# NVlabs/DREAM

Measured on AMD Instinct MI355X. Metric: frames/s DREAM-vgg-q 400x400 b=128 inference, higher is better.
Workload: dtype f32

## Files before the change

dream_amd/csrc/conv_wino4.hip:

```cpp
#include <type_traits>
#include <stdlib.h>
#include <dream_cdna4.h>
#include "common.h"
#include "pack_device.h"
#include "../../include/dream_hip.h"

#ifndef DREAM_W4_DIAG
#define DREAM_W4_DIAG 0
#endif
#ifndef DREAM_W4_STORE
#define DREAM_W4_STORE buffer_store_f32
#endif
#ifndef DREAM_W4_MIDBARRIER
#define DREAM_W4_MIDBARRIER 0
#endif
#ifndef DREAM_W4_STAGGER_N
#define DREAM_W4_STAGGER_N 0
#define DREAM_W4_STAGGER_PCT 0
#endif
#ifndef DREAM_W4_WAUX
#define DREAM_W4_WAUX 0
#endif
#ifndef DREAM_W4_XAUX
#define DREAM_W4_XAUX 0
#endif
#ifndef DREAM_W4_STAG_LX
#define DREAM_W4_STAG_LX 0
#endif
#ifndef DREAM_W4_RUNNING_WOFF
#define DREAM_W4_RUNNING_WOFF 1
#endif
#ifndef DREAM_W4_SETPRIO
#define DREAM_W4_SETPRIO 0
#endif

namespace {

struct Wino4Params {
    const float *x;
    const float *u;
    const float *scale;
    const float *shift;
    const float *residual;
    float *y;
    float *y_full;
    int B, H, W, Cin, Cout, CoutPad;
    int TY, TX;
    int ntiles;
    int nblk, blk_per_xcd;
    unsigned long long magic_tpi, magic_tx;
    int flags;
    int out_scale, out_oy, out_ox;
    int in_scale, in_oy, in_ox;
    int stagger_n, stagger_unit;
    int ymap;
};

constexpr int W4T = 16;
constexpr int W4P = 36;
#ifndef DREAM_W4_RING
#define DREAM_W4_RING 8
#endif
#ifndef DREAM_W4_NARROW_RING
#define DREAM_W4_NARROW_RING 18
#endif
#ifndef DREAM_W4_PAT_RING
#define DREAM_W4_PAT_RING 10
#endif
#ifndef DREAM_W4_PAT_S1OFF
#define DREAM_W4_PAT_S1OFF 8
#endif


template <bool NARROW>
struct W4Cfg {
    static constexpr int NW = NARROW ? 4 : 8;
    static constexpr int K = NARROW ? 8 : 16;
    static constexpr int Q = K / 4;
    static constexpr int KS = K / 4;
    static constexpr int PAD = 16 * NW;
    static constexpr int VPS = NARROW ? W4T * K : W4T * K + 16;
    static constexpr int VB = W4P * VPS;
    static constexpr int SROW = NARROW ? 14 : 25;
    static constexpr int QS = NARROW ? 7 : 6;
    static constexpr int SB = W4T * 6 * SROW * 4;
    static constexpr int RING = NARROW ? DREAM_W4_NARROW_RING : DREAM_W4_RING;
    static constexpr int AHEAD = RING - 2;
    static_assert(72 % RING == 0, "the weight ring must divide two chunks' positions");
    static constexpr bool PAIRS = NARROW && DREAM_W4_NARROW_PAIRS;
    static_assert(!PAIRS || RING % 2 == 0, "a ring of whole pairs");
    using vec = std::conditional_t<NARROW, f32x2, f32x4>;
};
template <bool NARROW>
DREAM_DEVICE int v4_slot(int q, int t) { return NARROW ? q ^ ((t >> 3) & 1) : q ^ ((t >> 2) & 2); }

DREAM_DEVICE f32x4 fma4(float c, f32x4 a, f32x4 b) {
    f32x4 r;
#pragma unroll
    for (int k = 0; k < 4; ++k) r[k] = __builtin_fmaf(c, a[k], b[k]);
    return r;
}

DREAM_DEVICE f32x4 sub4(f32x4 y, f32x4 x) { return pk_sub4(y, x); }
DREAM_DEVICE f32x4 bt_row(int j, const f32x4 *d) {
    switch (j) {
        case 0: return fma4(-2.0f, d[2], fma4(1.5f, sub4(d[3], d[1]), d[0] + d[4]));
        case 1: return fma4(2.5f, d[3], fma4(0.5f, d[2], sub4(d[4], d[1])));
        case 2: return fma4(0.5f, d[3], fma4(-2.5f, d[2], d[4] + d[1]));
        case 3: return fma4(2.0f, sub4(d[3], d[1]), sub4(d[4], d[2]));
        case 4: return fma4(-0.5f, sub4(d[3], d[1]), sub4(d[4], d[2]));
        default: return fma4(-2.0f, d[3], fma4(1.5f, sub4(d[4], d[2]), d[1] + d[5]));
    }
}

DREAM_DEVICE constexpr bool pat4_row_active(int pat, int i) { return pat == 0 || (((pat - 1) >> 1) == 0 ? i <= 4 : i >= 1); }
DREAM_DEVICE constexpr bool pat4_col_active(int pat, int j) { return pat == 0 || (((pat - 1) & 1) == 0 ? j <= 4 : j >= 1); }
DREAM_DEVICE constexpr bool pat4_active(int pat, int pp) { return pat4_row_active(pat, pp / 6) && pat4_col_active(pat, pp % 6); }
DREAM_DEVICE constexpr int pat4_count(int pat) { return pat == 0 ? 36 : 25; }
struct Pat4Table { int pos[36]; };
constexpr Pat4Table pat4_table(int pat) {
    Pat4Table t = {};
    int n = 0;
    for (int pp = 0; pp < 36; ++pp)
        if (pat4_active(pat, pp)) t.pos[n++] = pp;
    return t;
}
template <int PAT>
struct Pat4 { static constexpr Pat4Table table = pat4_table(PAT); };
#define pat4_pos(PAT, k) (Pat4<PAT>::table.pos[k])

template <int MODE, bool NARROW, int PAT = 0>
__global__ void __launch_bounds__(64 * W4Cfg<NARROW>::NW, 2) conv_wino4_kernel(const Wino4Params p) {
    using C = W4Cfg<NARROW>;
    using vec = typename C::vec;
    constexpr int W4K = C::K, W4NW = C::NW, V4PS = C::VPS, V4B = C::VB, S4ROW = C::SROW;
    constexpr int NPOS = pat4_count(PAT);
    constexpr int W4_RING = PAT ? DREAM_W4_PAT_RING : C::RING, W4_AHEAD = W4_RING - 2;
    static_assert((2 * NPOS) % W4_RING == 0, "the weight ring must divide two chunks' positions");
    DREAM_DYNAMIC_LDS(float, sV);
    const int tid = threadIdx.x;
    const int lane = tid & 63;
    const int wave = wave_index();
    const int item_id = wave * 48 + (lane < 48 ? lane : lane - 16);

    const int xcd = (int)(blockIdx.x & 7), J = (int)(gridDim.x >> 3);
    const int part = p.ymap ? xcd / p.ymap : xcd;
    const int blk_hi = (part + 1) * p.blk_per_xcd;
    const int blk_end = blk_hi < p.nblk ? blk_hi : p.nblk;
    int tb = part * p.blk_per_xcd + (int)(blockIdx.x >> 3);
    if (tb >= blk_end) return;
    const int n0 = (p.ymap ? xcd % p.ymap : (int)blockIdx.y) * (16 * W4NW);
    if (p.stagger_n > 1) {
        const unsigned w = blockIdx.x + blockIdx.y * gridDim.x;
        const int naps = (int)((w * 2654435761u >> 16) % (unsigned)p.stagger_n) * p.stagger_unit;
        for (int i = 0; i < naps; ++i) __builtin_amdgcn_s_sleep(127);
    }
    const int tiles_per_img = p.TY * p.TX;
    const int Si = PAT ? p.in_scale : 1;
    const size_t img_floats = (size_t)(Si * p.H) * (Si * p.W) * p.Cin;

    const int q1 = item_id % C::Q, r1 = (item_id / C::Q) % 6, t1 = (item_id / C::Q) / 6;
    const int s1_off = ((t1 * 6 + r1) * S4ROW + C::QS * q1) * 4;
    const int q2 = item_id % C::Q;
    const int j2 = NARROW ? (item_id >> 3) % 6 : (item_id >> 2) % 6;
    const int t2 = NARROW ? 4 * (item_id / 48) + ((item_id >> 1) & 3) : (item_id >> 2) / 6;
    const int s2_off = ((t2 * 6) * S4ROW + C::QS * q2 + j2) * 4;
    const int v2_off = j2 * V4PS + t2 * W4K + 4 * v4_slot<NARROW>(q2, t2);

    unsigned goff0;
    int item1 = t1 | (r1 << 8) | (q1 << 16);
    auto plan_item = [&](int tile0, int b0) {
        asm volatile("" : "+v"(item1));
        const int t = item1 & 255, r = (item1 >> 8) & 255, q = (item1 >> 16) & 255;
        const int tau = tile0 + t;
        const bool tv = tau < p.ntiles;
        const int b = div_magic40(tau, p.magic_tpi), rem = tau - b * tiles_per_img;
        const int ty = div_magic40(rem, p.magic_tx), tx = rem - ty * p.TX;
        const int gy = 4 * ty - 1 + r, x0 = 4 * tx - 1;
        const bool rok = tv & ((unsigned)gy < (unsigned)p.H);
        goff0 = PAT ? (unsigned)(((((b - b0) * Si * p.H + Si * gy + p.in_oy) * (Si * p.W) + Si * x0 + p.in_ox) * p.Cin + 4 * q) * 4)
                    : (unsigned)(((((b - b0) * p.H + gy) * p.W + x0) * p.Cin + 4 * q) * 4);
        item1 &= 0xffffff;
#pragma unroll
        for (int c = 0; c < 6; ++c) item1 |= (rok & ((unsigned)(x0 + c) < (unsigned)p.W)) ? (1 << (24 + c)) : 0;
    };
    const unsigned px_in = (unsigned)(Si * p.Cin * 4);
    auto item_offset = [&](int c) {
        if (DREAM_W4_DIAG & 16) {
            unsigned o = BUFFER_OOB;
            asm volatile("" : "+v"(o));
            return o;
        }
        return (item1 >> (24 + c)) & 1 ? goff0 + (unsigned)c * px_in : BUFFER_OOB;
    };
    auto block_tile0 = [&](int blk) { return blk < blk_end ? blk * W4T : p.ntiles; };
    auto block_xbuf = [&](int b0) {
        return make_buffer(p.x + (size_t)b0 * img_floats, ((size_t)(p.B - b0) * img_floats) * sizeof(float));
    };

    const int lt = lane & 15, lg = lane >> 4;
    const int a_off = NARROW ? lt * W4K + 4 * v4_slot<NARROW>(lg >> 1, lt) + 2 * (lg & 1) : lt * W4K + 4 * v4_slot<NARROW>(lg, lt);
    const unsigned b_lane = C::PAIRS ? (unsigned)(((wave * 16 + lt) * 16 + 4 * lg) * 4) : (unsigned)(((wave * 16 + lt) * W4K + C::KS * lg) * 4);
    const unsigned u_pos_stride = (unsigned)(p.CoutPad * W4K * 4);
    const BufferRsrc ubuf = make_buffer(p.u + (size_t)n0 * W4K, ((size_t)((p.Cin / W4K) * W4P + C::AHEAD) * p.CoutPad - (size_t)n0) * W4K * sizeof(float));

    f32x4 acc[W4P];
    const int nchunks = p.Cin / W4K;
    if (DREAM_W4_SETPRIO && wave >= W4NW / 2) __builtin_amdgcn_s_setprio(1);

    constexpr int BSTEP = C::PAIRS ? 2 : 1;
    std::conditional_t<C::PAIRS, f32x4, vec> bq[W4_RING / BSTEP];
    auto load_u = [&](unsigned soff) {
        if constexpr (C::PAIRS) return buffer_load_x4(ubuf, b_lane, soff);
        else if constexpr (NARROW) return buffer_load_x2(ubuf, b_lane, soff);
        else return buffer_load_x4_aux<DREAM_W4_WAUX>(ubuf, b_lane, soff);
    };
#pragma unroll
    for (int k = 0; k < W4_AHEAD; k += BSTEP) bq[k / BSTEP] = load_u((unsigned)pat4_pos(PAT, k) * u_pos_stride);
    unsigned woff = (unsigned)W4_AHEAD * u_pos_stride;
    DREAM_OPAQUE_SGPR(woff);

    f32x4 *const sV4 = (f32x4 *)sV;
    vec *const sVa = (vec *)sV;
    int vrd[2], vwr[2], s1p = (2 * V4B + s1_off) / 4, s2p = (2 * V4B + s2_off) / 4;
#pragma unroll
    for (int h = 0; h < 2; ++h) {
        vrd[h] = (h * V4B + a_off) / C::KS;
        vwr[h] = (h * V4B + v2_off) / 4;
        asm volatile("" : "+v"(vrd[h]), "+v"(vwr[h]));
    }
    asm volatile("" : "+v"(s1p), "+v"(s2p));
    f32x4 d[6];
    auto pass1_piece = [&](int j) { sV4[s1p + j] = bt_row(j, d); };
    auto pass2_read = [&](int r) { d[r] = sV4[s2p + r * S4ROW]; };
    auto pass2_piece = [&](int i, int h) { if (pat4_row_active(PAT, i)) sV4[vwr[h] + i * (6 * V4PS / 4)] = bt_row(i, d); };

    vec a[2][2];
    auto read_a = [&](int set, int k, int h) {
        const int p0 = pat4_pos(PAT, k), p1 = pat4_pos(PAT, k + 1 < NPOS ? k + 1 : k);
        if constexpr (NARROW) {
            a[set][0] = lds_read_unmerged(sVa + vrd[h] + p0 * V4PS / C::KS);
            a[set][1] = lds_read_unmerged(sVa + vrd[h] + p1 * V4PS / C::KS);
        } else {
            a[set][0] = sVa[vrd[h] + p0 * V4PS / C::KS];
            if (k + 1 < NPOS) a[set][1] = sVa[vrd[h] + p1 * V4PS / C::KS];
        }
    };

    int tile0 = block_tile0(tb);
    int b0 = div_magic40(tile0, p.magic_tpi);
    BufferRsrc xbuf = block_xbuf(b0);
    plan_item(tile0, b0);
#pragma unroll
    for (int c = 0; c < 6; ++c) d[c] = buffer_load_x4(xbuf, item_offset(c), 0u);
#pragma unroll
    for (int j = 0; j < 6; ++j) pass1_piece(j);
    __syncthreads();
#pragma unroll
    for (int r = 0; r < 6; ++r) pass2_read(r);
#pragma unroll
    for (int i = 0; i < 6; ++i) pass2_piece(i, 0);
    __syncthreads();

    auto chunk = [&](auto ph_tag, auto stag_tag, bool last, int c, int tile0n, int b0n) __attribute__((always_inline)) {
        constexpr int PH = decltype(ph_tag)::value;
        constexpr int STAG = decltype(stag_tag)::value;
#ifndef DREAM_W4_S1
#define DREAM_W4_S1 10
#define DREAM_W4_S2 13
#define DREAM_W4_LX 3
#endif
        constexpr int NSLOT = (NPOS + 1) / 2;
        constexpr int S1 = PAT ? NSLOT - DREAM_W4_PAT_S1OFF : DREAM_W4_S1, S2 = PAT ? S1 + 3 : DREAM_W4_S2;
        constexpr int LX = PAT ? 1 : DREAM_W4_LX;
        constexpr int LX0 = STAG ? DREAM_W4_STAG_LX : 0;
        static_assert(LX0 + LX <= S1, "the patch loads must be issued before pass 1");
        const unsigned coff = last ? 0u : (unsigned)((c + 1) * W4K * 4);
        const int cnext = last ? 0 : (c + 1) * W4P;
        if (PH == 1 && last) xbuf = block_xbuf(b0n);
        read_a(0, 0, PH);
        __builtin_amdgcn_sched_barrier(0);
#pragma unroll
        for (int s = 0; s < NSLOT; ++s) {
            const int k0 = 2 * s;
            const bool two = k0 + 1 < NPOS;
            const int pp = pat4_pos(PAT, k0), pp1 = pat4_pos(PAT, two ? k0 + 1 : k0);
            auto load_b = [&](int half) {
                if ((DREAM_W4_DIAG & 2) || (half && !two)) return;
                if (C::PAIRS && half) return;
                const int kn = k0 + half + W4_AHEAD;
                if constexpr (PAT == 0 && DREAM_W4_RUNNING_WOFF && !(DREAM_W4_DIAG & 32)) {
                    if (kn == NPOS && last) woff = 0u;
                    bq[(PH * NPOS + kn) % W4_RING / BSTEP] = load_u(woff);
                    woff += BSTEP * u_pos_stride;
                    DREAM_OPAQUE_SGPR(woff);
                } else {
                    const int spos = kn >= NPOS ? cnext + pat4_pos(PAT, kn - NPOS) : c * W4P + pat4_pos(PAT, kn);
                    bq[(PH * NPOS + kn) % W4_RING / BSTEP] = load_u((DREAM_W4_DIAG & 32) ? 0u : (unsigned)spos * u_pos_stride);
                }
            };
            auto load_x = [&](int col) { if (!(DREAM_W4_DIAG & 1)) d[col] = buffer_load_x4_aux<DREAM_W4_XAUX>(xbuf, item_offset(col), (DREAM_W4_DIAG & 64) ? 0u : coff); };
            auto pair = [&](int r) {
                const int i0 = (PH * NPOS + k0) % W4_RING, i1 = (PH * NPOS + k0 + 1) % W4_RING;
                if constexpr (C::PAIRS) {
                    acc[pp] = mfma_f32_16x16x4(a[s & 1][0][r], bq[i0 / 2][r], acc[pp]);
                    acc[pp1] = mfma_f32_16x16x4(a[s & 1][1][r], bq[i0 / 2][2 + r], acc[pp1]);
                } else {
                    acc[pp] = mfma_f32_16x16x4(a[s & 1][0][r], bq[i0][r], acc[pp]);
                    if (two) acc[pp1] = mfma_f32_16x16x4(a[s & 1][1][r], bq[i1][r], acc[pp1]);
                }
                __builtin_amdgcn_sched_barrier(0);
            };
            auto after = [&](int k) {
                if (k == 0) {
                    load_b(0);
                    if (s + 1 < NSLOT) read_a((s + 1) & 1, k0 + 2, PH);
                    if (PH == 1 && s == 0 && last) plan_item(tile0n, b0n);
                    if (s >= LX0 && s < LX0 + LX) { for (int c2 = 0; c2 < 3 / LX; ++c2) load_x((6 / LX) * (s - LX0) + c2); }
                    if (!(DREAM_W4_DIAG & 8) && s >= S1 && s < S1 + 3) pass1_piece(2 * (s - S1));
                    if (!(DREAM_W4_DIAG & 8) && s == S2) { pass2_read(0); pass2_read(1); }
                    if (!(DREAM_W4_DIAG & 8) && s > S2 && s <= S2 + 3) pass2_piece(2 * (s - S2 - 1), 1 - PH);
                } else if (k == 1) {
                    load_b(1);
                    if (s >= LX0 && s < LX0 + LX) { for (int c2 = 3 / LX; c2 < 6 / LX; ++c2) load_x((6 / LX) * (s - LX0) + c2); }
                    if (!(DREAM_W4_DIAG & 8) && s == S2) { pass2_read(2); pass2_read(3); }
                } else if (k == 2) {
                    if (!(DREAM_W4_DIAG & 8) && s >= S1 && s < S1 + 3) pass1_piece(2 * (s - S1) + 1);
                    if (!(DREAM_W4_DIAG & 8) && s == S2) { pass2_read(4); pass2_read(5); }
                    if (!(DREAM_W4_DIAG & 8) && s > S2 && s <= S2 + 3) pass2_piece(2 * (s - S2 - 1) + 1, 1 - PH);
                }
            };
            if constexpr (NARROW) {
                pair(0);
                after(0);
                after(1);
                pair(1);
                after(2);
            } else {
                pair(0);
                after(0);
                pair(1);
                after(1);
                pair(2);
                after(2);
                pair(3);
            }
            if (s == S1 + 2 && !(DREAM_W4_DIAG & 4)) {
                if (DREAM_W4_MIDBARRIER) __syncthreads();
                __builtin_amdgcn_sched_barrier(0);
            }
        }
        if (!(DREAM_W4_DIAG & 4)) __syncthreads();
    };
    const std::integral_constant<int, 0> ph0{};
    const std::integral_constant<int, 1> ph1{};

    constexpr bool pool = MODE == 1 || MODE == 4, both = MODE == 4, has_res = MODE == 2 || MODE == 3, mask = MODE == 3;
    auto epilogue = [&](auto site_tag, int tile0e, int b0e) {
        if (DREAM_W4_DIAG & 128) {
#pragma unroll
            for (int pp = 0; pp < W4P; ++pp)
                if (pat4_active(PAT, pp)) asm volatile("" :: "v"(acc[pp]));
            return;
        }
        const auto &e = *DREAM_KERNARG_SITE(p, decltype(site_tag)::value);
        const bool relu = (e.flags & DREAM_CONV_RELU) != 0;
        const bool late = MODE == 2 && (e.flags & DREAM_CONV_RES_AFTER_RELU) != 0;
        const int Ho = pool ? e.H / 2 : e.H, Wo = pool ? e.W / 2 : e.W, So = e.out_scale;
        const size_t out_img = (size_t)(So * Ho) * (So * Wo) * e.Cout;
        const unsigned px_b = (unsigned)(So * e.Cout * 4), row_b = (unsigned)(So * So * Wo * e.Cout * 4);
        const int ln = lane_id();
        const int lt = ln & 15, lg = ln >> 4;
        const int col = n0 + wave * 16 + lt;
        const bool cok = col < e.Cout;
        const float sc = (e.scale != nullptr && cok) ? e.scale[col] : 1.0f;
        const float sh = (e.shift != nullptr && cok) ? e.shift[col] : 0.0f;
        const BufferRsrc ybuf = make_buffer(e.y + (size_t)b0e * out_img, (DREAM_W4_DIAG & 256) ? 0 : (size_t)(e.B - b0e) * out_img * sizeof(float));
        const BufferRsrc rbuf = make_buffer(has_res ? e.residual + (size_t)b0e * out_img : e.y,
                                            has_res ? (size_t)(e.B - b0e) * out_img * sizeof(float) : 0);
        const size_t full_img = (size_t)e.H * e.W * e.Cout;
        const unsigned fpx_b = (unsigned)(e.Cout * 4), frow_b = (unsigned)(e.W * e.Cout * 4);
        const BufferRsrc fbuf = make_buffer(both ? e.y_full + (size_t)b0e * full_img : e.y, both ? (size_t)(e.B - b0e) * full_img * sizeof(float) : 0);
        const int tau0 = tile0e + lg * 4;
        int b = div_magic40(tau0, p.magic_tpi);
        const int rem = tau0 - b * tiles_per_img;
        int ty = div_magic40(rem, p.magic_tx), tx = rem - ty * p.TX;
        constexpr int NS = pool ? 2 : 4;
        unsigned basef[2][2];
        int limf[2][2];
        unsigned base4[2][2];
        int lim4[2][2];
        constexpr int FULL = pool ? 0x33 : 0xff;
#pragma unroll
        for (int rp = 0; rp < 2; ++rp)
#pragma unroll
            for (int h = 0; h < 2; ++h) {
                const bool tok = cok & ((tau0 + 2 * rp + h) < p.ntiles);
                const int oy = NS * ty, ox = NS * tx;
                base4[rp][h] = (unsigned)(((((b - b0e) * So * Ho + So * oy + e.out_oy) * (So * Wo) + So * ox + e.out_ox) * e.Cout + col) * 4);
                int m = 0;
#pragma unroll
                for (int i = 0; i < NS; ++i) m |= ((oy + i) < Ho ? 1 << i : 0) | ((ox + i) < Wo ? 16 << i : 0);
                lim4[rp][h] = tok ? m : 0;
                if (both) {
                    basef[rp][h] = (unsigned)(((((b - b0e) * e.H + 4 * ty) * e.W + 4 * tx) * e.Cout + col) * 4);
                    int mf = 0;
#pragma unroll
                    for (int i = 0; i < 4; ++i) mf |= ((4 * ty + i) < e.H ? 1 << i : 0) | ((4 * tx + i) < e.W ? 16 << i : 0);
                    limf[rp][h] = tok ? mf : 0;
                }
                const bool wrap_x = (tx + 1 == p.TX);
                const bool wrap_y = wrap_x & (ty + 1 == p.TY);
                tx = wrap_x ? 0 : tx + 1;
                ty = wrap_y ? 0 : (wrap_x ? ty + 1 : ty);
                b += wrap_y ? 1 : 0;
            }
        auto out_off4 = [&](int rp, int h, int i, int jj) {
            const bool inb = ((lim4[rp][h] >> i) & (lim4[rp][h] >> (4 + jj)) & 1) != 0;
            return inb ? base4[rp][h] + (unsigned)i * row_b + (unsigned)jj * px_b : BUFFER_OOB;
        };
        bool interior4[2];
#pragma unroll
        for (int rp = 0; rp < 2; ++rp) interior4[rp] = wave_all((lim4[rp][0] == FULL) & (lim4[rp][1] == FULL));
        auto load_col0 = [&](int rp, float (&r)[2][4]) {
            if (interior4[rp]) {
#pragma unroll
                for (int h = 0; h < 2; ++h)
#pragma unroll
                    for (int i = 0; i < 4; ++i) r[h][i] = buffer_load_f32(rbuf, base4[rp][h], (unsigned)i * row_b);
            } else {
#pragma unroll
                for (int h = 0; h < 2; ++h)
#pragma unroll
                    for (int i = 0; i < 4; ++i) r[h][i] = buffer_load_f32(rbuf, out_off4(rp, h, i, 0), 0u);
            }
        };
        float r0[2][4], r0n[2][4];
        if (has_res) load_col0(0, r0);
#pragma unroll
        for (int rp = 0; rp < 2; ++rp) {
            const unsigned (&base)[2] = base4[rp];
            auto out_off = [&](int h, int i, int jj) { return out_off4(rp, h, i, jj); };
            const bool all_interior = interior4[rp];
            auto fm = [](float c, f32x2 x, f32x2 y) { return __builtin_elementwise_fma(f32x2{c, c}, x, y); };
            f32x2 sA[6][4];
#pragma unroll
            for (int i = 0; i < 6; ++i) {
                f32x2 m[6];
#pragma unroll
                for (int j = 0; j < 6; ++j)
                    m[j] = pat4_active(PAT, 6 * i + j) ? f32x2{acc[6 * i + j][2 * rp], acc[6 * i + j][2 * rp + 1]} : f32x2{0.0f, 0.0f};
                const f32x2 t1 = pk_sub2(m[1], m[2]), t2 = m[1] + m[2];
                sA[i][0] = (m[0] + t2) + (m[3] + m[4]);
                sA[i][1] = fm(-2.0f, m[4], fm(0.5f, m[3], t1));
                sA[i][2] = fm(4.0f, m[4], fm(0.25f, m[3], t2));
                sA[i][3] = fm(-8.0f, m[4], fm(0.125f, m[3], t1)) + m[5];
            }
            auto finish = [&](float v, float rv) {
                if (has_res) v = mask ? (rv > 0.0f ? v : 0.0f) : (late ? v : v + rv);
                const float vr = fmaxf(v, 0.0f);
                v = relu ? vr : v;
                return (MODE == 2 && late) ? v + rv : v;
            };
            auto columns = [&](auto interior_tag, auto &rcur) {
                constexpr bool interior = decltype(interior_tag)::value;
                auto voff = [&](int h, int i, int j2) { return interior ? base[h] : out_off(h, i, j2); };
                auto soff = [&](int i, int j2) { return interior ? (unsigned)i * row_b + (unsigned)j2 * px_b : 0u; };
                float keep[2][2];
#pragma unroll
                for (int jj = 0; jj < 4; ++jj) {
                    float rnext[2][4];
                    if (has_res && jj == 3 && rp == 0) load_col0(1, r0n);
                    if (has_res && jj + 1 < 4) {
#pragma unroll
                        for (int h = 0; h < 2; ++h)
#pragma unroll
                            for (int i = 0; i < 4; ++i) rnext[h][i] = buffer_load_f32(rbuf, voff(h, i, jj + 1), soff(i, jj + 1));
                    }
                    const f32x2 t1 = pk_sub2(sA[1][jj], sA[2][jj]), t2 = sA[1][jj] + sA[2][jj];
                    f32x2 o4[4];
                    o4[0] = (sA[0][jj] + t2) + (sA[3][jj] + sA[4][jj]);
                    o4[1] = fm(-2.0f, sA[4][jj], fm(0.5f, sA[3][jj], t1));
                    o4[2] = fm(4.0f, sA[4][jj], fm(0.25f, sA[3][jj], t2));
                    o4[3] = fm(-8.0f, sA[4][jj], fm(0.125f, sA[3][jj], t1)) + sA[5][jj];
#pragma unroll
                    for (int i = 0; i < 4; ++i) o4[i] = o4[i] * f32x2{sc, sc} + f32x2{sh, sh};
#pragma unroll
                    for (int h = 0; h < 2; ++h) {
                        if (pool) {
                            float v[4];
#pragma unroll
                            for (int i = 0; i < 4; ++i) v[i] = finish(o4[i][h], 0.0f);
                            if (both) {
#pragma unroll
                                for (int i = 0; i < 4; ++i) {
                                    const bool inb = ((limf[rp][h] >> i) & (limf[rp][h] >> (4 + jj)) & 1) != 0;
                                    DREAM_W4_STORE(fbuf, v[i], inb ? basef[rp][h] + (unsigned)i * frow_b + (unsigned)jj * fpx_b : BUFFER_OOB, 0u);
                                }
                            }
                            if ((jj & 1) == 0) {
                                keep[h][0] = fmaxf(v[0], v[1]);
                                keep[h][1] = fmaxf(v[2], v[3]);
                            } else {
                                DREAM_W4_STORE(ybuf, fmaxf(keep[h][0], fmaxf(v[0], v[1])), voff(h, 0, jj >> 1), soff(0, jj >> 1));
                                DREAM_W4_STORE(ybuf, fmaxf(keep[h][1], fmaxf(v[2], v[3])), voff(h, 1, jj >> 1), soff(1, jj >> 1));
                            }
                        } else {
#pragma unroll
                            for (int i = 0; i < 4; ++i)
                                DREAM_W4_STORE(ybuf, finish(o4[i][h], has_res ? rcur[h][i] : 0.0f), voff(h, i, jj), soff(i, jj));
                        }
                    }
                    if (has_res && jj + 1 < 4) {
#pragma unroll
                        for (int h = 0; h < 2; ++h)
#pragma unroll
                            for (int i = 0; i < 4; ++i) rcur[h][i] = rnext[h][i];
                    }
                }
            };
            if (all_interior) columns(std::true_type{}, r0);
            else columns(std::false_type{}, r0);
            if (has_res && rp == 0) {
#pragma unroll
                for (int h = 0; h < 2; ++h)
#pragma unroll
                    for (int i = 0; i < 4; ++i) r0[h][i] = r0n[h][i];
            }
        }
    };

    auto run_blocks = [&](auto stag_tag) __attribute__((always_inline)) {
        while (true) {
            const int tile0n = block_tile0(tb + J);
            const int b0n = div_magic40(tile0n, p.magic_tpi);
            const f32x4 zero = {0.0f, 0.0f, 0.0f, 0.0f};
#pragma unroll
            for (int pp = 0; pp < W4P; ++pp)
                if (pat4_active(PAT, pp)) acc[pp] = zero;
            for (int c = 0; c < nchunks; c += 2) {
                chunk(ph0, stag_tag, false, c, tile0n, b0n);
                chunk(ph1, stag_tag, c + 2 == nchunks, c + 1, tile0n, b0n);
            }
            epilogue(stag_tag, tile0, b0);
            tb += J;
            if (tb >= blk_end) break;
            tile0 = tile0n;
            b0 = b0n;
        }
    };
    if constexpr (!NARROW && PAT == 0 && DREAM_W4_STAG_LX > 0) {
        if (wave >= W4NW / 2) run_blocks(std::integral_constant<int, 1>{});
        else run_blocks(std::integral_constant<int, 0>{});
    } else {
        run_blocks(std::integral_constant<int, 0>{});
    }
}

static_assert(W4Cfg<false>::K == 16 && W4Cfg<false>::PAD == 128 && W4Cfg<true>::K == 8 && W4Cfg<true>::PAD == 64 && W4P == 36,
              "pack_device.h assumes 16-channel chunks padded to 128 rows / 8-channel chunks padded to 64 rows, 36 positions");
__global__ void __launch_bounds__(256) wino4_pack_kernel(const float *w, float *u, int Cout, int Cin, int mode) {
    dream_pack::winograd4(w, u, Cout, Cin, mode, (int)blockIdx.x, (int)gridDim.x);
}

int g_max_workgroups4 = 0;
int g_stagger_n4 = -1, g_stagger_pct4 = 0;
int g_ymap4 = -1;

bool narrow_rows(int rows) { return rows <= W4Cfg<true>::PAD; }
struct PackShape { int k, rows_pad, ahead; };
PackShape pack_shape(int rows) {
    if (narrow_rows(rows)) return {W4Cfg<true>::K, W4Cfg<true>::PAD, W4Cfg<true>::AHEAD};
    return {W4Cfg<false>::K, (rows + W4Cfg<false>::PAD - 1) / W4Cfg<false>::PAD * W4Cfg<false>::PAD, W4Cfg<false>::AHEAD};
}

template <int MODE, bool NARROW, int PAT = 0>
int launch_wino4(const Wino4Params &p, void *stream) {
    using C = W4Cfg<NARROW>;
    void (*kernel)(const Wino4Params) = conv_wino4_kernel<MODE, NARROW, PAT>;
    const size_t lds = ((size_t)2 * C::VB + C::SB) * sizeof(float);
    if (dream_allow_full_lds((const void *)kernel)) return 2;
    const int ny = (p.Cout + 16 * C::NW - 1) / (16 * C::NW);
    const int resident = g_max_workgroups4 > 0 ? g_max_workgroups4 : (NARROW ? 512 : 256);
    Wino4Params q = p;
    dim3 grid;
    if (g_ymap4 && !NARROW && (ny == 2 || ny == 4) && resident >= 64 && p.nblk >= resident) {
        q.ymap = ny;
        q.blk_per_xcd = (p.nblk + 8 / ny - 1) / (8 / ny);
        grid = dim3((unsigned)(resident / 8 * 8), 1u);
    } else {
        int gx = resident / ny / 8 * 8;
        if (gx < 8) gx = 8;
        if (gx > (p.nblk + 7) / 8 * 8) gx = (p.nblk + 7) / 8 * 8;
        grid = dim3((unsigned)gx, (unsigned)ny);
    }
    hipLaunchKernelGGL(kernel, grid, dim3(64 * C::NW), lds, (hipStream_t)stream, q);
    DREAM_LAUNCH_OK();
    return 0;
}

template <bool NARROW>
int launch_wino4_mode(const Wino4Params &p, int mode, void *stream) {
    switch (mode) {
        case 0: return launch_wino4<0, NARROW>(p, stream);
        case 1: return launch_wino4<1, NARROW>(p, stream);
        case 2: return launch_wino4<2, NARROW>(p, stream);
        case 4: return launch_wino4<4, NARROW>(p, stream);
        default: return launch_wino4<3, NARROW>(p, stream);
    }
}

}

extern "C" size_t dream_conv3x3_winograd4_weight_floats(int rows, int cols) {
    const PackShape ps = pack_shape(rows);
    return ((size_t)(cols / ps.k) * W4P + ps.ahead) * ps.rows_pad * ps.k;
}

extern "C" int dream_conv3x3_winograd4_set_channel_block_pinning(int on) {
    DREAM_REQUIRE(on >= -1 && on <= 1, "winograd F(4x4): pinning %d", on);
    g_ymap4 = on;
    return 0;
}

extern "C" int dream_conv3x3_winograd4_set_stagger(int phases, int percent) {
    DREAM_REQUIRE(phases <= 1024 && percent >= 0 && percent <= 400, "winograd F(4x4): stagger %d phases over %d %%", phases, percent);
    g_stagger_n4 = phases < 0 ? -1 : (phases > 1 ? phases : 0);
    g_stagger_pct4 = percent;
    return 0;
}

extern "C" int dream_conv3x3_winograd4_set_max_workgroups(int n) {
    DREAM_REQUIRE(n >= 0, "winograd F(4x4): max workgroups %d", n);
    g_max_workgroups4 = n;
    return 0;
}

extern "C" int dream_pack_conv3x3_winograd4_weight(const float *w_oihw, float *u, int Cout, int Cin, int mode, void *stream) {
    DREAM_REQUIRE(w_oihw && u && Cout > 0 && Cin > 0 && (mode == 0 || mode == 1), "winograd F(4x4) pack: bad arguments");
    const int rows = mode == 0 ? Cout : Cin, cols = mode == 0 ? Cin : Cout;
    const PackShape ps = pack_shape(rows);
    DREAM_REQUIRE(cols % (2 * ps.k) == 0, "winograd F(4x4) pack: %d input channels, must be a multiple of %d", cols, 2 * ps.k);
    const size_t total = (size_t)(cols / ps.k) * ps.rows_pad * ps.k;
    size_t grid = (total + 255) / 256;
    if (grid > 4096) grid = 4096;
    hipLaunchKernelGGL(wino4_pack_kernel, dim3((unsigned)grid), dim3(256), 0, (hipStream_t)stream, w_oihw, u, Cout, Cin, mode);
    DREAM_LAUNCH_OK();
    if (dream_zero_words(u + (size_t)(cols / ps.k) * W4P * ps.rows_pad * ps.k, (size_t)ps.ahead * ps.rows_pad * ps.k * sizeof(float), (hipStream_t)stream))
        return 2;
    return 0;
}

namespace {

int wino4_setup(Wino4Params &p, const float *x, const float *u_packed, const float *scale, const float *shift, const float *residual,
                float *y, int B, int H, int W, int Cin, int Cout, int flags, int out_scale, int in_scale = 1) {
    DREAM_REQUIRE(x && u_packed && y, "winograd F(4x4) conv: null pointer");
    DREAM_REQUIRE(B > 0 && H > 0 && W > 0 && Cin > 0 && Cout > 0, "winograd F(4x4) conv: bad shape B=%d H=%d W=%d Cin=%d Cout=%d", B, H, W, Cin, Cout);
    const PackShape ps = pack_shape(Cout);
    DREAM_REQUIRE(Cin % (2 * ps.k) == 0, "winograd F(4x4) conv: Cin=%d must be a multiple of %d", Cin, 2 * ps.k);
    const size_t span_imgs = (size_t)W4T / ((size_t)((H + 3) / 4) * ((W + 3) / 4)) + 2;
    DREAM_REQUIRE(span_imgs * in_scale * in_scale * H * W * (size_t)Cin * sizeof(float) < ((size_t)1 << 31) &&
                  span_imgs * out_scale * out_scale * H * W * (size_t)Cout * sizeof(float) < ((size_t)1 << 31),
                  "winograd F(4x4) conv: image too large for 32-bit offsets");
    p.x = x; p.u = u_packed; p.scale = scale; p.shift = shift; p.residual = residual; p.y = y; p.y_full = nullptr;
    p.B = B; p.H = H; p.W = W; p.Cin = Cin; p.Cout = Cout;
    p.CoutPad = Cout <= ps.rows_pad ? ps.rows_pad : (Cout + ps.rows_pad - 1) / ps.rows_pad * ps.rows_pad;
    DREAM_REQUIRE(((size_t)(Cin / ps.k) * W4P + ps.ahead) * (size_t)p.CoutPad * ps.k * sizeof(float) < ((size_t)1 << 31), "winograd F(4x4) conv: weights too large");
    p.TY = (H + 3) / 4; p.TX = (W + 3) / 4;
    const long ntiles = (long)B * p.TY * p.TX;
    DREAM_REQUIRE(ntiles < ((long)1 << 24), "winograd F(4x4) conv: %ld tiles, the tile decomposition handles < 2^24", ntiles);
    p.ntiles = (int)ntiles;
    p.nblk = (p.ntiles + W4T - 1) / W4T;
    p.blk_per_xcd = (p.nblk + 7) / 8;
    p.magic_tpi = (((unsigned long long)1 << 40) + (unsigned long long)(p.TY * p.TX) - 1) / (unsigned long long)(p.TY * p.TX);
    p.magic_tx = (((unsigned long long)1 << 40) + (unsigned long long)p.TX - 1) / (unsigned long long)p.TX;
    p.flags = flags;
    p.out_scale = out_scale; p.out_oy = 0; p.out_ox = 0;
    p.in_scale = in_scale; p.in_oy = 0; p.in_ox = 0;
    p.ymap = 0;
    if (g_stagger_n4 < 0) {
        const char *e = getenv("DREAM_W4_STAGGER");
        int n = DREAM_W4_STAGGER_N, pct = DREAM_W4_STAGGER_PCT;
        if (e != nullptr && sscanf(e, "%d,%d", &n, &pct) != 2) { n = DREAM_W4_STAGGER_N; pct = DREAM_W4_STAGGER_PCT; }
        g_stagger_n4 = n > 1 ? n : 0;
        g_stagger_pct4 = pct;
    }
    {
        const double chunk_cycles = narrow_rows(Cout) ? 7000.0 : 13500.0;
        const double block_naps = (double)(Cin / ps.k) * chunk_cycles / 8128.0;
        p.stagger_n = g_stagger_n4;
        p.stagger_unit = g_stagger_n4 > 1 ? (int)(block_naps * g_stagger_pct4 / 100.0 / g_stagger_n4 + 0.5) : 0;
        if (p.stagger_n > 1 && p.stagger_unit < 1) p.stagger_unit = 1;
    }
    if (g_ymap4 < 0) {
        const char *e = getenv("DREAM_W4_YMAP");
        g_ymap4 = (e != nullptr && e[0] == '0') ? 0 : 1;
    }
    return 0;
}

}

extern "C" int dream_conv3x3_winograd4_nhwc_f32(const float *x, const float *u_packed, const float *scale, const float *shift,
                                                const float *residual, float *y, int B, int H, int W, int Cin, int Cout, int flags,
                                                void *stream) {
    DREAM_REQUIRE((flags & ~(DREAM_CONV_RELU | DREAM_CONV_POOL2 | DREAM_CONV_RELUMASK | DREAM_CONV_RES_AFTER_RELU)) == 0, "winograd F(4x4) conv: unsupported flags 0x%x", flags);
    DREAM_REQUIRE(!(flags & DREAM_CONV_RES_AFTER_RELU) || (residual != nullptr && !(flags & (DREAM_CONV_POOL2 | DREAM_CONV_RELUMASK))),
                  "winograd F(4x4) conv: residual-after-ReLU needs a residual and excludes the fused pool / the ReLU mask");
    DREAM_REQUIRE(!(flags & DREAM_CONV_POOL2) || (residual == nullptr && H >= 2 && W >= 2), "winograd F(4x4) conv: fused max-pool takes no residual");
    DREAM_REQUIRE(!(flags & DREAM_CONV_RELUMASK) || residual != nullptr, "winograd F(4x4) conv: ReLU mask without a mask tensor");
    Wino4Params p;
    if (int rc = wino4_setup(p, x, u_packed, scale, shift, residual, y, B, H, W, Cin, Cout, flags, 1)) return rc;
    const int mode = (flags & DREAM_CONV_POOL2) ? 1 : (flags & DREAM_CONV_RELUMASK) ? 3 : (residual != nullptr ? 2 : 0);
    return narrow_rows(Cout) ? launch_wino4_mode<true>(p, mode, stream) : launch_wino4_mode<false>(p, mode, stream);
}

extern "C" int dream_conv3x3_winograd4_pool_both_nhwc_f32(const float *x, const float *u_packed, const float *scale, const float *shift,
                                                          float *y_full, float *y_pool, int B, int H, int W, int Cin, int Cout, int flags,
                                                          void *stream) {
    DREAM_REQUIRE((flags & ~DREAM_CONV_RELU) == 0, "winograd F(4x4) conv + pool: unsupported flags 0x%x", flags);
    DREAM_REQUIRE(y_full != nullptr && y_pool != nullptr && H >= 2 && W >= 2, "winograd F(4x4) conv + pool: null output or map too small");
    Wino4Params p;
    if (int rc = wino4_setup(p, x, u_packed, scale, shift, nullptr, y_pool, B, H, W, Cin, Cout, flags, 1)) return rc;
    p.y_full = y_full;
    return narrow_rows(Cout) ? launch_wino4_mode<true>(p, 4, stream) : launch_wino4_mode<false>(p, 4, stream);
}

extern "C" size_t dream_convT4x4_winograd4_weight_floats(int Cout, int Cin) { return 4 * dream_conv3x3_winograd4_weight_floats(Cout, Cin); }

extern "C" int dream_pack_convT4x4_winograd4_weight(const float *wT, float *u4, float *scratch, int Cin, int Cout, int mode, void *stream) {
    DREAM_REQUIRE(wT && u4 && scratch && Cin > 0 && Cout > 0 && (mode == 0 || mode == 1), "winograd F(4x4) convT pack: bad arguments");
    if (int rc = dream_convT4x4_phase_weights(wT, scratch, Cin, Cout, mode, stream)) return rc;
    const int rows = mode == 0 ? Cout : Cin, cols = mode == 0 ? Cin : Cout;
    const size_t per_u = dream_conv3x3_winograd4_weight_floats(rows, cols);
    for (int ph = 0; ph < 4; ++ph)
        if (int rc = dream_pack_conv3x3_winograd4_weight(scratch + (size_t)ph * Cout * Cin * 9, u4 + ph * per_u, rows, cols, 0, stream)) return rc;
    return 0;
}

extern "C" int dream_conv4x4s2_winograd4_nhwc_f32(const float *dy, const float *u4, float *dx, int B, int H, int W, int Cout, int Cin,
                                                  void *stream) {
    DREAM_REQUIRE(Cin > 64, "winograd F(4x4) conv4x4s2: needs more than 64 output channels (the wide workgroup shape), got %d", Cin);
    Wino4Params p;
    if (int rc = wino4_setup(p, dy, u4, nullptr, nullptr, nullptr, dx, B, H, W, Cout, Cin, 0, 1, 2)) return rc;
    const size_t per_u = dream_conv3x3_winograd4_weight_floats(Cin, Cout);
    for (int ph = 0; ph < 4; ++ph) {
        p.u = u4 + ph * per_u;
        p.in_oy = ph >> 1; p.in_ox = ph & 1;
        p.residual = ph == 0 ? nullptr : dx;
        int rc;
        switch (ph) {
            case 0: rc = launch_wino4<0, false, 4>(p, stream); break;
            case 1: rc = launch_wino4<2, false, 3>(p, stream); break;
            case 2: rc = launch_wino4<2, false, 2>(p, stream); break;
            default: rc = launch_wino4<2, false, 1>(p, stream); break;
        }
        if (rc) return rc;
    }
    return 0;
}

extern "C" int dream_conv_transpose4x4s2_winograd4_nhwc_f32(const float *x, const float *u4, const float *scale, const float *shift,
                                                            float *y, int B, int H, int W, int Cin, int Cout, int flags, void *stream) {
    DREAM_REQUIRE((flags & ~DREAM_CONV_RELU) == 0, "winograd F(4x4) convT: unsupported flags 0x%x", flags);
    DREAM_REQUIRE(Cout > 64, "winograd F(4x4) convT: needs more than 64 output channels (the wide workgroup shape), got %d", Cout);
    Wino4Params p;
    if (int rc = wino4_setup(p, x, u4, scale, shift, nullptr, y, B, H, W, Cin, Cout, flags, 2)) return rc;
    const size_t per_u = dream_conv3x3_winograd4_weight_floats(Cout, Cin);
    for (int ph = 0; ph < 4; ++ph) {
        p.u = u4 + ph * per_u;
        p.out_oy = ph >> 1; p.out_ox = ph & 1;
        int rc;
        switch (ph) {
            case 0: rc = launch_wino4<0, false, 1>(p, stream); break;
            case 1: rc = launch_wino4<0, false, 2>(p, stream); break;
            case 2: rc = launch_wino4<0, false, 3>(p, stream); break;
            default: rc = launch_wino4<0, false, 4>(p, stream); break;
        }
        if (rc) return rc;
    }
    return 0;
}
```

Measured before the change: 2564.

## Stage Winograd F(4x4) epilogue through LDS slab for 16-byte output stores

Adds a wide epilogue for plain and pooled modes that applies the output transform, writes results into a per-wave LDS slab, then reads back four contiguous channels per lane and issues dwordx4 buffer stores. This replaces per-element scalar stores and is meant to cut store instruction count and improve write coalescing. It costs extra LDS per workgroup and LDS round trips with wave-level syncs. It is selected automatically when Cout is a multiple of 4 and the output is 16-byte aligned.

After: 2567 (median of 3 runs). About the same (+0.1%).

```diff
diff --git a/dream_amd/csrc/conv_wino4.hip b/dream_amd/csrc/conv_wino4.hip
--- a/dream_amd/csrc/conv_wino4.hip
+++ b/dream_amd/csrc/conv_wino4.hip
@@ -7,6 +7,9 @@
 
 #ifndef DREAM_W4_DIAG
 #define DREAM_W4_DIAG 0
+#endif
+#ifndef DREAM_W4_WIDE_STORES
+#define DREAM_W4_WIDE_STORES 1
 #endif
 #ifndef DREAM_W4_STORE
 #define DREAM_W4_STORE buffer_store_f32
@@ -90,7 +93,20 @@
     static constexpr bool PAIRS = NARROW && DREAM_W4_NARROW_PAIRS;
     static_assert(!PAIRS || RING % 2 == 0, "a ring of whole pairs");
     using vec = std::conditional_t<NARROW, f32x2, f32x4>;
+    static constexpr int SLAB_TS = 80;
+    static constexpr int SLAB = W4T * SLAB_TS;
 };
+template <int MODE, bool NARROW>
+constexpr bool w4_wide_stores() { return DREAM_W4_WIDE_STORES && (MODE == 0 || MODE == 1); }
+template <bool NARROW>
+constexpr size_t w4_lds_bytes(bool wide) {
+    using C = W4Cfg<NARROW>;
+    return ((size_t)2 * C::VB + C::SB + (wide ? C::NW * C::SLAB : 0)) * sizeof(float);
+}
+static_assert(w4_lds_bytes<false>(true) <= 160 * 1024, "wide shape: LDS");
+static_assert(2 * w4_lds_bytes<true>(true) <= 160 * 1024, "narrow shape: two workgroups per CU");
+static_assert((2 * W4Cfg<false>::VB + W4Cfg<false>::SB) % 4 == 0 && (2 * W4Cfg<true>::VB + W4Cfg<true>::SB) % 4 == 0 && W4Cfg<false>::SLAB % 4 == 0,
+              "the slab's b128 reads are 16-byte aligned");
 template <bool NARROW>
 DREAM_DEVICE int v4_slot(int q, int t) { return NARROW ? q ^ ((t >> 3) & 1) : q ^ ((t >> 2) & 2); }
 
@@ -129,8 +145,9 @@
 struct Pat4 { static constexpr Pat4Table table = pat4_table(PAT); };
 #define pat4_pos(PAT, k) (Pat4<PAT>::table.pos[k])
 
-template <int MODE, bool NARROW, int PAT = 0>
+template <int MODE, bool NARROW, int PAT = 0, bool WIDE = false>
 __global__ void __launch_bounds__(64 * W4Cfg<NARROW>::NW, 2) conv_wino4_kernel(const Wino4Params p) {
+    static_assert(!WIDE || w4_wide_stores<MODE, NARROW>(), "the dwordx4 epilogue exists for MODE 0 and 1");
     using C = W4Cfg<NARROW>;
     using vec = typename C::vec;
     constexpr int W4K = C::K, W4NW = C::NW, V4PS = C::VPS, V4B = C::VB, S4ROW = C::SROW;
@@ -356,6 +373,112 @@
     const std::integral_constant<int, 1> ph1{};
 
     constexpr bool pool = MODE == 1 || MODE == 4, both = MODE == 4, has_res = MODE == 2 || MODE == 3, mask = MODE == 3;
+    auto epilogue_wide = [&](const auto &e, bool relu, int tile0e, int b0e) {
+        using Cw = W4Cfg<NARROW>;
+        constexpr int TS = Cw::SLAB_TS, NS = pool ? 2 : 4, FULL = pool ? 0x33 : 0xff;
+        const int Ho = pool ? e.H / 2 : e.H, Wo = pool ? e.W / 2 : e.W, So = e.out_scale;
+        const size_t out_img = (size_t)(So * Ho) * (So * Wo) * e.Cout;
+        const unsigned px_b = (unsigned)(So * e.Cout * 4), row_b = (unsigned)(So * So * Wo * e.Cout * 4);
+        int ln = lane_id();
+        asm volatile("" : "+v"(ln));
+        const int lt = ln & 15, lg = ln >> 4;
+        const int col = n0 + wave * 16 + lt;
+        const bool cok = col < e.Cout;
+        const float sc = (e.scale != nullptr && cok) ? e.scale[col] : 1.0f;
+        const float sh = (e.shift != nullptr && cok) ? e.shift[col] : 0.0f;
+        const BufferRsrc ybuf = make_buffer(e.y + (size_t)b0e * out_img, (DREAM_W4_DIAG & 256) ? 0 : (size_t)(e.B - b0e) * out_img * sizeof(float));
+        const int tau = tile0e + (ln >> 2), c4 = n0 + wave * 16 + 4 * (ln & 3);
+        const int b = div_magic40(tau, p.magic_tpi), rem = tau - b * tiles_per_img;
+        const int ty = div_magic40(rem, p.magic_tx), tx = rem - ty * p.TX;
+        const int oy = NS * ty, ox = NS * tx;
+        const unsigned base = (unsigned)(((((b - b0e) * So * Ho + So * oy + e.out_oy) * (So * Wo) + So * ox + e.out_ox) * e.Cout + c4) * 4);
+        int lim = 0;
+#pragma unroll
+        for (int i = 0; i < NS; ++i) lim |= ((oy + i) < Ho ? 1 << i : 0) | ((ox + i) < Wo ? 16 << i : 0);
+        lim = ((c4 < e.Cout) & (tau < p.ntiles)) ? lim : 0;
+        const bool interior = wave_all(lim == FULL);
+        int swr = 2 * V4B + Cw::SB + wave * Cw::SLAB + 4 * lg * TS + lt;
+        int srd = (2 * V4B + Cw::SB + wave * Cw::SLAB + (ln >> 2) * TS + 4 * (ln & 3)) / 4;
+        asm volatile("" : "+v"(swr), "+v"(srd));
+        auto slab_turn = [&]() {
+            asm volatile("" ::: "memory");
+            (void)wave_bcast0(0);
+            asm volatile("" ::: "memory");
+        };
+        auto fm = [](float c, f32x2 x, f32x2 y) { return __builtin_elementwise_fma(f32x2{c, c}, x, y); };
+        auto finish = [&](float v) {
+            const float vr = fmaxf(v, 0.0f);
+            return relu ? vr : v;
+        };
+        f32x2 sA[2][6][4];
+#pragma unroll
+        for (int i = 0; i < 6; ++i)
+#pragma unroll
+            for (int rp = 0; rp < 2; ++rp) {
+                f32x2 m[6];
+#pragma unroll
+                for (int j = 0; j < 6; ++j)
+                    m[j] = pat4_active(PAT, 6 * i + j) ? f32x2{acc[6 * i + j][2 * rp], acc[6 * i + j][2 * rp + 1]} : f32x2{0.0f, 0.0f};
+                const f32x2 t1 = pk_sub2(m[1], m[2]), t2 = m[1] + m[2];
+                sA[rp][i][0] = (m[0] + t2) + (m[3] + m[4]);
+                sA[rp][i][1] = fm(-2.0f, m[4], fm(0.5f, m[3], t1));
+                sA[rp][i][2] = fm(4.0f, m[4], fm(0.25f, m[3], t2));
+                sA[rp][i][3] = fm(-8.0f, m[4], fm(0.125f, m[3], t1)) + m[5];
+            }
+        auto columns = [&](auto interior_tag) {
+            constexpr bool inside = decltype(interior_tag)::value;
+            float keep[2][2][2];
+#pragma unroll
+            for (int jj = 0; jj < 4; ++jj) {
+#pragma unroll
+                for (int rp = 0; rp < 2; ++rp) {
+                    const f32x2 t1 = pk_sub2(sA[rp][1][jj], sA[rp][2][jj]), t2 = sA[rp][1][jj] + sA[rp][2][jj];
+                    f32x2 o4[4];
+                    o4[0] = (sA[rp][0][jj] + t2) + (sA[rp][3][jj] + sA[rp][4][jj]);
+                    o4[1] = fm(-2.0f, sA[rp][4][jj], fm(0.5f, sA[rp][3][jj], t1));
+                    o4[2] = fm(4.0f, sA[rp][4][jj], fm(0.25f, sA[rp][3][jj], t2));
+                    o4[3] = fm(-8.0f, sA[rp][4][jj], fm(0.125f, sA[rp][3][jj], t1)) + sA[rp][5][jj];
+#pragma unroll
+                    for (int i = 0; i < 4; ++i) o4[i] = o4[i] * f32x2{sc, sc} + f32x2{sh, sh};
+#pragma unroll
+                    for (int h = 0; h < 2; ++h) {
+                        float *const tile = sV + swr + (2 * rp + h) * TS;
+                        if (pool) {
+                            float v[4];
+#pragma unroll
+                            for (int i = 0; i < 4; ++i) v[i] = finish(o4[i][h]);
+                            if ((jj & 1) == 0) {
+                                keep[rp][h][0] = fmaxf(v[0], v[1]);
+                                keep[rp][h][1] = fmaxf(v[2], v[3]);
+                            } else {
+                                tile[0] = fmaxf(keep[rp][h][0], fmaxf(v[0], v[1]));
+                                tile[16] = fmaxf(keep[rp][h][1], fmaxf(v[2], v[3]));
+                            }
+                        } else {
+#pragma unroll
+                            for (int i = 0; i < 4; ++i) tile[16 * i] = finish(o4[i][h]);
+                        }
+                    }
+                }
+                if (pool && (jj & 1) == 0) continue;
+                const int js = pool ? jj >> 1 : jj;
+                slab_turn();
+#pragma unroll
+                for (int i = 0; i < NS; ++i) {
+                    const f32x4 v = sV4[srd + 4 * i];
+                    if (inside) {
+                        buffer_store_x4(ybuf, v, base, (unsigned)i * row_b + (unsigned)js * px_b);
+                    } else {
+                        const bool inb = ((lim >> i) & (lim >> (4 + js)) & 1) != 0;
+                        buffer_store_x4(ybuf, v, inb ? base + (unsigned)i * row_b + (unsigned)js * px_b : BUFFER_OOB, 0u);
+                    }
+                }
+                slab_turn();
+            }
+        };
+        if (interior) columns(std::true_type{});
+        else columns(std::false_type{});
+    };
     auto epilogue = [&](auto site_tag, int tile0e, int b0e) {
         if (DREAM_W4_DIAG & 128) {
 #pragma unroll
@@ -366,6 +489,10 @@
         const auto &e = *DREAM_KERNARG_SITE(p, decltype(site_tag)::value);
         const bool relu = (e.flags & DREAM_CONV_RELU) != 0;
         const bool late = MODE == 2 && (e.flags & DREAM_CONV_RES_AFTER_RELU) != 0;
+        if constexpr (WIDE) {
+            epilogue_wide(e, relu, tile0e, b0e);
+            return;
+        }
         const int Ho = pool ? e.H / 2 : e.H, Wo = pool ? e.W / 2 : e.W, So = e.out_scale;
         const size_t out_img = (size_t)(So * Ho) * (So * Wo) * e.Cout;
         const unsigned px_b = (unsigned)(So * e.Cout * 4), row_b = (unsigned)(So * So * Wo * e.Cout * 4);
@@ -574,11 +701,15 @@
     return {W4Cfg<false>::K, (rows + W4Cfg<false>::PAD - 1) / W4Cfg<false>::PAD * W4Cfg<false>::PAD, W4Cfg<false>::AHEAD};
 }
 
-template <int MODE, bool NARROW, int PAT = 0>
+template <int MODE, bool NARROW, int PAT = 0, bool WIDE = false>
 int launch_wino4(const Wino4Params &p, void *stream) {
     using C = W4Cfg<NARROW>;
-    void (*kernel)(const Wino4Params) = conv_wino4_kernel<MODE, NARROW, PAT>;
-    const size_t lds = ((size_t)2 * C::VB + C::SB) * sizeof(float);
+    if constexpr (!WIDE && w4_wide_stores<MODE, NARROW>()) {
+        if (p.Cout % 4 == 0 && ((size_t)p.y & 15) == 0) return launch_wino4<MODE, NARROW, PAT, true>(p, stream);
+    }
+    void (*kernel)(const Wino4Params) = conv_wino4_kernel<MODE, NARROW, PAT, WIDE>;
+    constexpr size_t lds = w4_lds_bytes<NARROW>(WIDE);
+    static_assert(lds * (NARROW ? 2 : 1) <= 160 * 1024, "winograd F(4x4): LDS per CU");
     if (dream_allow_full_lds((const void *)kernel)) return 2;
     const int ny = (p.Cout + 16 * C::NW - 1) / (16 * C::NW);
     const int resident = g_max_workgroups4 > 0 ? g_max_workgroups4 : (NARROW ? 512 : 256);
```
